# facebookresearch/omni3d

Hardware: AMD Instinct MI355X
Metric: images/sec train DLA34_FPN b=4/GPU (higher is better)
Workload: dtype f32; 1 GPU; cubercnn_DLA34_FPN train step, batch 4/GPU, synthetic Omni3D 512x512 (8 GT/img), fwd+10 losses+bwd+allreduce+divergence guard+SGD, random-init weights; global_batch=4, image=512x512, parallelism=dp1 (flat-bucket RCCL all-reduce)

## Files before the change

### include/omni3d_hip.h

```cpp
#ifndef OMNI3D_HIP_H
#define OMNI3D_HIP_H

#ifdef __cplusplus
extern "C" {
#endif


int omni_iou_box3d(const float* boxes1, int N, const float* boxes2, int M, const int* valid1, float* vol,
                   float* iou, int* overflow, void* stream);

int omni_iou_box3d_pairs(const float* boxes1, const float* boxes2, const int* idx1, const int* idx2,
                         long long npairs, const int* valid1, float* vol, float* iou, int* overflow,
                         void* stream);

int omni_iou_box3d_pairs_algo(const float* boxes1, const float* boxes2, const int* idx1, const int* idx2,
                              long long npairs, const int* valid1, float* vol, float* iou, int* overflow,
                              int lanes_per_pair, void* stream);

int omni_box3d_validity(const float* boxes, int N, float eps_coplanar, float eps_nonzero, int* valid,
                        int* counts, void* stream);

int omni_nms3d(const float* verts, const float* score, const int* cls, const int* count, int B, int S, float iou_thr,
               int class_agnostic, float eps_coplanar, float eps_nonzero, float* iou, int* keep, int* order, int* new_count,
               int* overflow, void* stream);
// ... 57 lines not shown

int omni_conv2d_fwd_multi_det(const void* const* xs, const int* cs, int nsrc, const float* w, const float* bias, float* out, int N, int H,
                              int W, int K, int ldo, int relu, int tile, int splits_req, float* stats, int stats_rows, int* nblk_out,
                              float* ws, long long ws_floats, int* ctr, int n_ctr, long long* plan, void* stream);
int omni_conv2d_dgrad_det(const float* dy, const float* w, float* dx, int N, int H, int W, int C, int K, int R, int S,
                          int stride, int pad, int lddy, int lddx, int accumulate, int tile, int splits, float* ws,
                          long long ws_floats, int* ctr, int n_ctr, long long* plan, void* stream);
int omni_conv2d_wgrad_det(const float* x, const float* dy, float* dw, int N, int H, int W, int C, int K, int R, int S,
                          int stride, int pad, int ldx, int lddy, int accumulate, int tile, float* ws, long long ws_floats,
                          int* ctr, int n_ctr, long long* plan, void* stream);

int omni_gemm_batched_split(const float* A, const float* B, float* out, int batch, int M, int N, int K, int terms, void* stream);
int omni_conv2d_s2_dgrad(const float* dy, const float* w, float* dx, int N, int H, int W, int C, int K, int lddy, int lddx,
                         int accumulate, void* stream);
int omni_conv2d_wgrad_multi_det(const void* const* xs, const int* cs, int nsrc, const float* dy, float* dw, int N, int H, int W, int K,
                                int lddy, int accumulate, int tile, float* ws, long long ws_floats, int* ctr, int n_ctr, long long* plan,
                                void* stream);


int omni_bn_fwd_algo(const float* x, const float* partial, int nblk, const float* gamma, const float* beta, const float* residual,
                     float* y, long long ldy, float* running_mean, float* running_var, float* mean_rstd, float* scale_shift,
                     double* ws, int P, int C, float eps, float momentum, int relu, int fuse_rows, void* stream);
int omni_bn_bwd_algo(const float* x, const float* dy, long long lddy, const float* y, const float* gamma, const float* mean_rstd,
                     const float* partial, int nblk, float* dx, float* dres, const float* res_carry, long long ldc, float* dgamma,
                     float* dbeta, double* ws, float* coef, int P, int C, int relu, int accumulate_param_grads, int fuse_rows,
                     void* stream);

int omni_bn_apply(const float* x, const float* scale_shift, const float* residual, float* y, int P, int C,
                  int relu, void* stream);

int omni_bn_frozen_fwd(const float* x, const float* gamma, const float* beta, const float* running_mean, const float* running_var,
                       float eps, const float* residual, float* y, int P, int C, int relu, void* stream);
int omni_bn_frozen_bwd(const float* x, const float* dy, long long lddy, const float* y, const float* gamma, const float* beta,
                       const float* running_mean, const float* running_var, float eps, float* dx, float* dres, const float* res_carry,
                       long long ldc, float* dgamma, float* dbeta, float* ws, long long ws_floats, int P, int C, int relu,
                       int accumulate_param_grads, void* stream);

int omni_maxpool2_fwd(const float* x, float* y, int N, int H, int W, int C, void* stream);
int omni_maxpool2_bwd(const float* x, const float* dy, float* dx, int N, int H, int W, int C, void* stream);

int omni_grouped_conv2d_fwd(const float* x, const float* w, float* out, int N, int H, int W, int C, int K, int R, int S, int stride,
                            int pad, int groups, void* stream);
int omni_grouped_conv2d_dgrad(const float* dy, const float* w, float* dx, int N, int H, int W, int C, int K, int R, int S, int stride,
                              int pad, int groups, void* stream);
int omni_grouped_conv2d_wgrad(const float* x, const float* dy, float* dw, int N, int H, int W, int C, int K, int R, int S, int stride,
                              int pad, int groups, void* stream);

int omni_dwconv_fwd(const float* x, const float* w, float* y, int N, int H, int W, int C, int R, int stride, int pad, void* stream);
int omni_dwconv_dgrad(const float* dy, const float* w, float* dx, int N, int H, int W, int C, int R, int stride, int pad, void* stream);
int omni_dwconv_wgrad(const float* x, const float* dy, float* dw, int N, int H, int W, int C, int R, int stride, int pad, void* stream);

int omni_avgpool2_fwd(const float* x, float* y, int N, int H, int W, int C, void* stream);
int omni_avgpool2_bwd(const float* dy, float* dx, int N, int H, int W, int C, void* stream);

int omni_subsample2_fwd(const float* x, float* y, int N, int H, int W, int C, void* stream);
int omni_subsample2_bwd(const float* dy, float* dx, int N, int H, int W, int C, void* stream);

int omni_upsample2_add(const float* lat, const float* top, float* out, int N, int H, int W, int C,
                       void* stream);
int omni_upsample2_bwd(const float* dout, float* dtop, int N, int H, int W, int C, void* stream);

int omni_wino_out_carry(const float* M, const float* carry, long long ldc, float* y, int N, int H, int W, int K, int tile, void* stream);
int omni_maxpool2_bwd_carry(const float* x, const float* dy, long long lddy, const float* carry, long long ldc, float* dx, int N, int H,
                            int W, int C, void* stream);
int omni_subsample2_bwd_carry(const float* dy, const float* carry, long long ldc, float* dx, int N, int H, int W, int C, void* stream);
int omni_upsample2_bwd_carry(const float* dout, const float* carry, long long ldc, float* dtop, int N, int H, int W, int C,
                             void* stream);

int omni_preprocess(const unsigned char* img, float* out, int N, int H, int W, int PH, int PW, float m0,
                    float m1, float m2, float s0, float s1, float s2, void* stream);
int omni_preprocess_masked(const unsigned char* img, const int* image_hw, float* out, int N, int H, int W, int PH, int PW,
                           float m0, float m1, float m2, float s0, float s1, float s2, void* stream);
int omni_preprocess_multi(const void* const* imgs, const int* image_hw, float* out, int N, int H, int W, int PH, int PW, float m0,
                          float m1, float m2, float s0, float s1, float s2, void* stream);


int omni_topk_rows(const float* keys, int rows, int n, long long pitch, int estride, int k, float* out_val,
                   int* out_idx, void* stream);
int omni_topk_segments(const float* keys, int rows, long long pitch, int estride, int nseg, const int* seg_off,
                       const int* seg_n, int k, float* out_val, int* out_idx, void* stream);

int omni_nms_sorted(const float* boxes, const int* counts, const int* valid, int Q, int nmax, float iou_thr,
                    unsigned long long* mask_ws, int* keep, void* stream);


int omni_pairwise_iou(const float* boxes1, int N, const float* boxes2, int M, int mode, float* out, void* stream);


int omni_rpn_finalize_labels(const float* anchors, int A, int B, const int* gt_off, const float* ign,
                             const int* ign_off, const signed char* match_label, const int* gt_best_idx,
                             const float* pos_val, const int* pos_idx, const float* neg_val, const int* neg_idx,
                             int kpos, int kneg, int batch_per_image, float ignore_thresh, signed char* labels,
                             int* counts, void* stream);

int omni_rpn_gather_logits(const void* const* level_ptrs, const int* level_hw, int nlev, int B, float* logits,
                           void* stream);

int omni_rpn_head16_fwd(const void* const* t, const long long* pix, int nlev, const float* w_obj, const float* b_obj,
                        const float* w_del, const float* b_del, const void* const* y, void* stream);
int omni_rpn_head16_dgrad(const void* const* dy, const void* const* t, const long long* pix, int nlev, const float* w_obj,
                          const float* w_del, int relu_mask, const void* const* dt, void* stream);
int omni_rpn_head16_wgrad(const void* const* dy, const void* const* t, const long long* pix, int nlev, float* partial,
                          int partial_rows, float* dw_obj, float* db_obj, float* dw_del, float* db_del, int accumulate, void* stream);

int omni_rpn_loss_fwd(const void* const* level_ptrs, const int* level_hw, int nlev, int B, const float* anchors,
                      const signed char* labels, const int* matched_idx, const float* gt, const int* gt_off,
                      double* sums, void* stream);
int omni_rpn_loss_bwd(const void* const* level_ptrs, const void* const* dlevel_ptrs, const int* level_hw, int nlev,
                      int B, const float* anchors, const signed char* labels, const int* matched_idx,
                      const float* gt, const int* gt_off, const float* g_cls, const float* g_loc, float inv_norm,
                      void* stream);

int omni_rpn_loss_plain_fwd(const void* const* level_ptrs, const int* level_hw, int nlev, int B, const float* anchors,
                            const signed char* labels, const int* matched_idx, const float* gt, const int* gt_off,
                            double* sums, void* stream);
int omni_rpn_loss_plain_bwd(const void* const* level_ptrs, const void* const* dlevel_ptrs, const int* level_hw, int nlev,
                            int B, const float* anchors, const signed char* labels, const int* matched_idx,
                            const float* gt, const int* gt_off, const float* g_cls, const float* g_loc, float inv_norm,
                            void* stream);

int omni_rpn_decode(const void* const* level_ptrs, const int* level_hw, int nlev, int B, int Ktot,
                    const int* slot_level, const int* idx, const float* anchors, const int* image_hw,
                    float scale_clamp, float min_size, float* boxes, int* valid, void* stream);

int omni_rpn_mask_scores(const float* scores, const int* keep, long long n, float* masked, void* stream);
int omni_rpn_collect(const float* boxes, const float* top_v, const int* top_i, int B, int N, int P, float* prop,
                     int* count, void* stream);

int omni_rpn_match_draw(const float* anchors, int A, const float* gt, const int* gt_off, int B, int G, float thr_lo,
                        float thr_hi, int l0, int l1, int l2, int allow_low_quality, const float* expo, long long* draw_state,
                        int* ticket, float eps, float* matched_val, int* matched_idx, signed char* match_label, int* gt_best_bits,
                        int* gt_best_idx, float* key_pos, float* key_neg, void* stream);
int omni_roi_sample_draw(const float* prop_boxes, const int* prop_count, int B, int pmax, const float* gt, const int* gt_cls,
                         const int* gt_off, const float* ign, const int* ign_off, const float* expo, long long* draw_state, int* ticket,
                         float iou_thr, float ignore_thresh, float eps, int num_classes, int batch_per_image, int nfg_max,
                         int append_gt, float* out_boxes, int* out_cls, int* out_gt, float* out_iou, int* out_counts, int* out_row,
                         int first, float* first_boxes, int* first_cls, int* first_row, void* stream);


int omni_roi_levels(const float* rois, int R, int min_level, int max_level, float canonical_size,
                    int canonical_level, int* levels, void* stream);

int omni_roi_align_fwd(const void* const* level_ptrs, const int* level_hw, const float* level_scale, int nlev,
                       const float* rois, const int* batch_idx, const int* levels, int R, int P, int C,
                       float* out, void* stream);
int omni_roi_align_fwd_mode(const void* const* level_ptrs, const int* level_hw, const float* level_scale, int nlev,
                            const float* rois, const int* batch_idx, const int* levels, int R, int P, int C, int aligned, float* out,
                            void* stream);
int omni_roi_align_bwd_mode(const void* const* dlevel_ptrs, const int* level_hw, const float* level_scale, int nlev,
                            const float* rois, const int* batch_idx, const int* levels, int R, int P, int C, int aligned,
                            const float* dout, void* stream);
int omni_roi_pool_fwd(const void* const* level_ptrs, const int* level_hw, const float* level_scale, int nlev, const float* rois,
                      const int* batch_idx, const int* levels, int R, int P, int C, float* out, int* argmax, void* stream);
int omni_roi_pool_bwd(const void* const* dlevel_ptrs, const int* level_hw, const float* level_scale, int nlev, const int* batch_idx,
                      const int* levels, int R, int P, int C, const float* dout, const int* argmax, void* stream);
int omni_roi_align_fwd2(const void* const* level_ptrs, const int* level_hw, const float* level_scale, int nlev,
                        const float* rois, const int* batch_idx, const int* levels, int R, int P, int C, float* out,
                        float* out2, int per_image, int first, void* stream);
int omni_roi_align_bwd(const void* const* dlevel_ptrs, const int* level_hw, const float* level_scale, int nlev,
                       const float* rois, const int* batch_idx, const int* levels, int R, int P, int C,
                       const float* dout, void* stream);
int omni_roi_align_bwd2(const void* const* dlevel_ptrs, const int* level_hw, const float* level_scale, int nlev,
                        const float* rois, const int* batch_idx, const int* levels, int R, int P, int C,
                        const float* dout, const float* dout2, int per_image, int first, void* stream);
int omni_roi_align_bwd_det(const void* const* dlevel_ptrs, const int* level_hw, const float* level_scale, int nlev, int B,
                           const float* rois, const int* batch_idx, const int* levels, int R, int P, int C, const float* dout,
// ... 185 lines not shown
```

### omni3d_amd/csrc/select_nms.hip

```cpp
#include <device_rt.h>

namespace {

constexpr int TOPK_THREADS = 1024;
constexpr int TOPK_MAXK = 8192;

__device__ __forceinline__ unsigned score_bits(float f) {
    unsigned u = __float_as_uint(f);
    if (f != f) u = 0u;
    else if (f == 0.f) u = 0x80000000u;
    else u = (u & 0x80000000u) ? ~u : (u | 0x80000000u);
    return u;
}
__device__ __forceinline__ unsigned long long key_of_bits(unsigned u, int idx) {
    return ((unsigned long long)u << 32) | (unsigned long long)(0xFFFFFFFFu - (unsigned)idx);
}
__device__ __forceinline__ unsigned long long make_key(float f, int idx) { return key_of_bits(score_bits(f), idx); }
__device__ __forceinline__ void store_key(unsigned long long* sel, int slot, unsigned u, int idx) {
    unsigned* w = reinterpret_cast<unsigned*>(sel + slot);
    w[0] = 0xFFFFFFFFu - (unsigned)idx;
    w[1] = u;
}
__device__ __forceinline__ bool key_ge(unsigned u, int idx, unsigned thi, unsigned tlo) {
    return u > thi || (u == thi && (0xFFFFFFFFu - (unsigned)idx) >= tlo);
// ... 189 lines not shown
                for (int q = 0; q < 4; ++q) {
                    const unsigned long long key = ((unsigned long long)cu[q] << 32) | cl[q];
                    if (cv[q] && key >= thr) sel[atomicAdd(&s_count, 1)] = key;
                }
            }
            for (int i = kk + t; i < kpad; i += TOPK_THREADS) sel[i] = 0ull;
            selected = true;
        }
    }

    if (!selected) {
        unsigned long long thr = 0ull;
        if (kk < n) {
            if (t == 0) { R.prefix = 0ull; R.need = kk; }
            __syncthreads();
            for (int pass = 7; pass >= 0; --pass) {
                if (t < 256) R.hist[t] = 0u;
                __syncthreads();
                const unsigned long long prefix = R.prefix;
                const int shift = pass * 8;
                if (NPT > 0 && !PREF) {
                    int tt = t, nn = n;
                    OMNI_OPAQUE_V(tt);
                    OMNI_OPAQUE_S(nn);
                    const unsigned phi = (unsigned)(prefix >> 32), plo = (unsigned)prefix;
                    const bool hi = pass >= 4;
                    const int sh = hi ? shift - 32 : shift;
#pragma unroll
                    for (int j = 0; j < NPT; ++j) {
                        if (j * TOPK_THREADS >= nn) break;
                        const int i = j * TOPK_THREADS + tt;
                        const unsigned w = hi ? ku[j] : (0xFFFFFFFFu - (unsigned)i), pw = hi ? phi : plo;
                        bool todo = i < nn && (hi || ku[j] == phi);
                        if (sh < 24) todo = todo && ((w >> (sh + 8)) == (pw >> (sh + 8)));
                        count_digit(R.hist, todo, (w >> sh) & 255u);
                    }
                } else {
                    for (int base = 0; base < n; base += TOPK_THREADS) {
                        const int i = base + t;
                        bool todo = false;
                        unsigned digit = 0u;
                        if (i < n) {
                            const unsigned long long key = make_key(row[(long)i * estride], i);
                            todo = (pass == 7) || ((key >> (shift + 8)) == (prefix >> (shift + 8)));
                            digit = (unsigned)(key >> shift) & 255u;
                        }
                        count_digit(R.hist, todo, digit);
                    }
                }
                __syncthreads();
                radix_pick_bin(R, shift);
                __syncthreads();
                if (R.done) break;
            }
            thr = R.prefix;
        }
        if (t == 0) s_count = 0;
        for (int i = t; i < kpad; i += TOPK_THREADS) sel[i] = 0ull;
        __syncthreads();
        if (NPT > 0 && !PREF) {
            int tt = t;
            OMNI_OPAQUE_V(tt);
            const unsigned thi = (unsigned)(thr >> 32), tlo = (unsigned)thr;
#pragma unroll
            for (int j = 0; j < NPT; ++j) {
                if (j * TOPK_THREADS >= n) break;
                const int i = j * TOPK_THREADS + tt;
                if (i < n && key_ge(ku[j], i, thi, tlo)) {
                    const int slot = atomicAdd(&s_count, 1);
                    if (slot < TOPK_MAXK) store_key(sel, slot, ku[j], i);
                }
            }
        } else {
            for (int i = t; i < n; i += TOPK_THREADS) {
                const unsigned long long key = make_key(row[(long)i * estride], i);
                if (key >= thr) {
                    const int slot = atomicAdd(&s_count, 1);
                    if (slot < TOPK_MAXK) sel[slot] = key;
                }
            }
        }
    }
    __syncthreads();
    for (int size = 2; size <= kpad; size <<= 1) {
        for (int stride = size >> 1; stride > 0; stride >>= 1) {
            for (int i = t; i < (kpad >> 1); i += TOPK_THREADS) {
                const int lo = 2 * i - (i & (stride - 1));
                const int hi = lo + stride;
                const bool desc = ((lo & size) == 0);
                const unsigned long long a = sel[lo], b = sel[hi];
                if ((a < b) == desc) { sel[lo] = b; sel[hi] = a; }
            }
            __syncthreads();
        }
    }
    for (int i = t; i < k; i += TOPK_THREADS) {
        const long o = (long)blockIdx.x * k + i;
        if (i < kk) { out_val[o] = key_value(sel[i]); out_idx[o] = key_index(sel[i]); }
        else { out_val[o] = -INFINITY; out_idx[o] = -1; }
    }
}

__global__ void __launch_bounds__(256) nms_mask_kernel(const float* __restrict__ boxes, const int* __restrict__ counts,
                                                       int nmax, int words, float thr,
                                                       unsigned long long* __restrict__ mask) {
    const int lane = threadIdx.x & 63, wave = threadIdx.x >> 6;
    const int q = blockIdx.z, rb = blockIdx.y * 4 + wave, cb = blockIdx.x;
    const int n = counts ? counts[q] : nmax;
    if ((int)blockIdx.y * 4 > cb || cb * 64 >= n) return;
    __shared__ float cbx[64 * 4];
    const float* B = boxes + (long)q * nmax * 4;
    if (wave == 0) {
        const int j = cb * 64 + lane;
        if (j < n) {
            cbx[lane * 4 + 0] = B[j * 4 + 0]; cbx[lane * 4 + 1] = B[j * 4 + 1];
            cbx[lane * 4 + 2] = B[j * 4 + 2]; cbx[lane * 4 + 3] = B[j * 4 + 3];
        }
    }
    __syncthreads();
    if (cb < rb || rb * 64 >= n) return;
    const int i = rb * 64 + lane;
    if (i >= n) return;
    const float x1 = B[i * 4 + 0], y1 = B[i * 4 + 1], x2 = B[i * 4 + 2], y2 = B[i * 4 + 3];
    const float ai = (x2 - x1) * (y2 - y1);
    unsigned long long bits = 0ull;
    const int jmax = (n - cb * 64) < 64 ? (n - cb * 64) : 64;
    for (int jj = (rb == cb ? lane + 1 : 0); jj < jmax; ++jj) {
        const float u1 = cbx[jj * 4 + 0], v1 = cbx[jj * 4 + 1], u2 = cbx[jj * 4 + 2], v2 = cbx[jj * 4 + 3];
        const float w = fmaxf(fminf(x2, u2) - fmaxf(x1, u1), 0.f);
        const float h = fmaxf(fminf(y2, v2) - fmaxf(y1, v1), 0.f);
        const float inter = w * h;
        const float aj = (u2 - u1) * (v2 - v1);
        const float iou = inter / (ai + aj - inter);
        if (iou > thr) bits |= (1ull << jj);
    }
    mask[((long)q * nmax + i) * words + cb] = bits;
}

constexpr int SCAN_WAVES = 16;
template <int NMS_SCAN_WAVES>
__global__ void __launch_bounds__(64 * NMS_SCAN_WAVES) nms_scan_kernel(const unsigned long long* __restrict__ mask,
                                                                       const int* __restrict__ counts, const int* __restrict__ valid,
                                                                       int nmax, int words, int* __restrict__ keep) {
    constexpr int RPW = 64 / NMS_SCAN_WAVES;
    const int q = blockIdx.x, tid = threadIdx.x, lane = tid & 63, wave = tid >> 6;
    const int n = counts ? counts[q] : nmax;
    __shared__ unsigned long long s_alive;
    __shared__ unsigned long long s_next[NMS_SCAN_WAVES];
    for (int i = n + tid; i < nmax; i += 64 * NMS_SCAN_WAVES) keep[(long)q * nmax + i] = 0;
    const int nchunks = (n + 63) / 64;
    unsigned long long rw0[RPW], rw1[RPW], diag = 0ull, acc0 = 0ull, acc1 = 0ull, removed_c = 0ull;
    int okv = 0;
    auto fetch = [&](int c) {
#pragma unroll
        for (int rr = 0; rr < RPW; ++rr) {
            const int row = c * 64 + wave * RPW + rr;
            const long rowbase = ((long)q * nmax + row) * words;
            const int w0 = lane, w1 = 64 + lane;
            rw0[rr] = (row < n && w0 > c && w0 < words && w0 * 64 < n) ? mask[rowbase + w0] : 0ull;
            rw1[rr] = (words > 64 && row < n && w1 > c && w1 < words && w1 * 64 < n) ? mask[rowbase + w1] : 0ull;
        }
        if (wave == 0) {
            const int i = c * 64 + lane;
            diag = i < n ? mask[((long)q * nmax + i) * words + c] : 0ull;
            okv = (i < n && (valid == nullptr || valid[(long)q * nmax + i] != 0)) ? 1 : 0;
        }
    };
    if (nchunks > 0) fetch(0);
    for (int c = 0; c < nchunks; ++c) {
        if (wave == 0) {
            const int i = c * 64 + lane;
            unsigned long long alive = __ballot(okv != 0) & ~removed_c;
            for (int r = 0; r < 64; ++r) {
                const unsigned long long d = __shfl(diag, r, 64);
                if ((alive >> r) & 1ull) alive &= ~d;
            }
            if (i < n) keep[(long)q * nmax + i] = (int)((alive >> lane) & 1ull);
            if (lane == 0) s_alive = alive;
        }
        __syncthreads();
        const unsigned long long alive = s_alive;
#pragma unroll
        for (int rr = 0; rr < RPW; ++rr) {
            if ((alive >> (wave * RPW + rr)) & 1ull) { acc0 |= rw0[rr]; acc1 |= rw1[rr]; }
        }
        const int nw = c + 1;
        const unsigned long long mine = __shfl(nw < 64 ? acc0 : acc1, nw & 63, 64);
        if (lane == 0) s_next[wave] = mine;
        if (c + 1 < nchunks) fetch(c + 1);
        __syncthreads();
        if (wave == 0) {
            removed_c = 0ull;
#pragma unroll
            for (int k = 0; k < NMS_SCAN_WAVES; ++k) removed_c |= s_next[k];
        }
    }
}

inline void launch_topk(int blocks, int nmax, const float* keys, const SegP& seg, long pitch, int estride, int k, float* out_val,
                        int* out_idx, hipStream_t st) {
    if (nmax <= TOPK_NPT * TOPK_THREADS && k <= TOPK_PREFILTER_K)
        hipLaunchKernelGGL(HIP_KERNEL_NAME(topk_rows_kernel<TOPK_NPT, true>), dim3(blocks), dim3(TOPK_THREADS), 0, st, keys, seg, pitch, estride,
                           k, out_val, out_idx);
    else if (nmax <= TOPK_NPT * TOPK_THREADS)
        hipLaunchKernelGGL(HIP_KERNEL_NAME(topk_rows_kernel<TOPK_NPT, false>), dim3(blocks), dim3(TOPK_THREADS), 0, st, keys, seg, pitch, estride,
                           k, out_val, out_idx);
    else
        hipLaunchKernelGGL(HIP_KERNEL_NAME(topk_rows_kernel<0, false>), dim3(blocks), dim3(TOPK_THREADS), 0, st, keys, seg, pitch, estride, k,
                           out_val, out_idx);
}

}

extern "C" {

int omni_topk_rows(const float* keys, int rows, int n, long long pitch, int estride, int k, float* out_val, int* out_idx,
                   void* stream) {
    if (rows < 0 || n < 0 || k <= 0 || k > TOPK_MAXK || estride <= 0) return OMNI_ERR_ARG;
    if (rows == 0) return OMNI_OK;
    SegP seg;
    seg.S = 1;
    for (int i = 0; i < TOPK_MAXSEG; ++i) { seg.off[i] = 0; seg.n[i] = n; }
    launch_topk(rows, n, keys, seg, (long)pitch, estride, k, out_val, out_idx, (hipStream_t)stream);
    return omni_launch_status();
}

int omni_topk_segments(const float* keys, int rows, long long pitch, int estride, int nseg, const int* seg_off,
                       const int* seg_n, int k, float* out_val, int* out_idx, void* stream) {
    if (rows < 0 || nseg <= 0 || nseg > TOPK_MAXSEG || k <= 0 || k > TOPK_MAXK || estride <= 0) return OMNI_ERR_ARG;
    if (rows == 0) return OMNI_OK;
    SegP seg;
    seg.S = nseg;
    for (int i = 0; i < TOPK_MAXSEG; ++i) {
        seg.off[i] = i < nseg ? seg_off[i] : 0;
        seg.n[i] = i < nseg ? seg_n[i] : 0;
        if (seg.off[i] < 0 || seg.n[i] < 0) return OMNI_ERR_ARG;
    }
    int nmax = 0;
    for (int i = 0; i < nseg; ++i) nmax = seg.n[i] > nmax ? seg.n[i] : nmax;
    launch_topk(rows * nseg, nmax, keys, seg, (long)pitch, estride, k, out_val, out_idx, (hipStream_t)stream);
    return omni_launch_status();
}

int omni_nms_sorted(const float* boxes, const int* counts, const int* valid, int Q, int nmax, float iou_thr,
                    unsigned long long* mask_ws, int* keep, void* stream) {
    if (Q < 0 || nmax < 0 || nmax > 8192) return OMNI_ERR_ARG;
    if (Q == 0 || nmax == 0) return OMNI_OK;
    const int words = (nmax + 63) / 64;
    hipStream_t st = (hipStream_t)stream;
    hipLaunchKernelGGL(nms_mask_kernel, dim3(words, (words + 3) / 4, Q), dim3(256), 0, st, boxes, counts, nmax, words, iou_thr,
                       mask_ws);
    hipLaunchKernelGGL(HIP_KERNEL_NAME(nms_scan_kernel<SCAN_WAVES>), dim3(Q), dim3(64 * SCAN_WAVES), 0, st, (const unsigned long long*)mask_ws,
                       counts, valid, nmax, words, keep);
    return omni_launch_status();
}

}
```

### omni3d_amd/cubercnn/modeling/proposal_generator/rpn.py

```python
import math

import torch
from torch import nn

from .... import functional as HF
from ....d2.config import configurable
from ....d2.structures import Boxes, Instances
from ....kernels import det, select
from ..anchors import build_anchor_generator
from ..layers import Conv2d
from ..registries import PROPOSAL_GENERATOR_REGISTRY, RPN_HEAD_REGISTRY

CL = torch.channels_last


@RPN_HEAD_REGISTRY.register()
class StandardRPNHead(nn.Module):

    @configurable
    def __init__(self, *, in_channels, num_anchors, box_dim=4, conv_dims=(-1,)):
        super().__init__()
        assert len(conv_dims) == 1 and num_anchors == 3 and box_dim == 4, "hot path: A=3 anchors per location"
        out_channels = in_channels if conv_dims[0] == -1 else conv_dims[0]
        self.conv = Conv2d(in_channels, out_channels, kernel_size=3, stride=1, padding=1)
# ... 53 lines not shown
            raise NotImplementedError("MI355X hot path: L1 anchor regression (BBOX_REG_LOSS_TYPE smooth_l1, SMOOTH_L1_BETA 0: Base.yaml / "
                                      "upstream defaults); the reference's IoUness losses only evaluate smooth_l1 as well (rpn.py:258-271)")
        if objectness_uncertainty.lower() not in ("iouness", "none"):
            raise NotImplementedError(f"MODEL.RPN.OBJECTNESS_UNCERTAINTY '{objectness_uncertainty}': 'IoUness' (Base.yaml:55) and 'none'")
        self.plain_objectness = objectness_uncertainty.lower() == "none"
        self.pending_logs = {}
        self.injected = None
        self.last = None

    @classmethod
    def from_config(cls, cfg, input_shape):
        in_features = cfg.MODEL.RPN.IN_FEATURES
        shapes = [input_shape[f] for f in in_features]
        return {
            "in_features": in_features, "min_box_size": cfg.MODEL.PROPOSAL_GENERATOR.MIN_SIZE,
            "nms_thresh": cfg.MODEL.RPN.NMS_THRESH, "batch_size_per_image": cfg.MODEL.RPN.BATCH_SIZE_PER_IMAGE,
            "positive_fraction": cfg.MODEL.RPN.POSITIVE_FRACTION,
            "loss_weight": {"loss_rpn_cls": cfg.MODEL.RPN.LOSS_WEIGHT,
                            "loss_rpn_loc": cfg.MODEL.RPN.BBOX_REG_LOSS_WEIGHT * cfg.MODEL.RPN.LOSS_WEIGHT},
            "box_reg_loss_type": cfg.MODEL.RPN.BBOX_REG_LOSS_TYPE, "smooth_l1_beta": cfg.MODEL.RPN.SMOOTH_L1_BETA,
            "pre_nms_topk": (cfg.MODEL.RPN.PRE_NMS_TOPK_TRAIN, cfg.MODEL.RPN.PRE_NMS_TOPK_TEST),
            "post_nms_topk": (cfg.MODEL.RPN.POST_NMS_TOPK_TRAIN, cfg.MODEL.RPN.POST_NMS_TOPK_TEST),
            "anchor_generator": build_anchor_generator(cfg, shapes),
            "anchor_thresholds": cfg.MODEL.RPN.IOU_THRESHOLDS, "anchor_labels": cfg.MODEL.RPN.IOU_LABELS,
            "head": build_rpn_head(cfg, shapes), "ignore_thresh": cfg.MODEL.RPN.IGNORE_THRESHOLD,
            "objectness_uncertainty": cfg.MODEL.RPN.OBJECTNESS_UNCERTAINTY,
        }

    @torch.no_grad()
    def label_and_sample_anchors(self, anchors, targets):
        B, A = targets.B, anchors.shape[0]
        E = self.injected["E"].to(anchors.device).float().contiguous() if (self.injected is not None and "E" in self.injected) else None
        if E is None and self.__dict__.get("_draw") is None:
            from ....kernels.glue import DrawState
            self.__dict__["_draw"] = DrawState()
        thr = self.anchor_thresholds
        m = det.rpn_match(anchors, targets.gt, targets.gt_off, E, (thr[0], thr[-1]), self.anchor_labels, True, draw=self.__dict__.get("_draw"), B=B)
        kpos = max(int(self.batch_size_per_image * self.positive_fraction), 1)
        kv, ki = select.topk_rows(m["keys"], max(kpos, self.batch_size_per_image))
        pv, pi = kv[:B, :kpos].contiguous(), ki[:B, :kpos].contiguous()
        nv, ni = kv[B:, :self.batch_size_per_image].contiguous(), ki[B:, :self.batch_size_per_image].contiguous()
        labels, counts = det.rpn_finalize_labels(anchors, targets.gt_off, targets.ign, targets.ign_off, m, pv, pi, nv, ni,
                                                 self.batch_size_per_image, self.ignore_thresh)
        return labels, m["matched_idx"]

    def losses(self, levels, anchors, labels, matched_idx, targets):
        B = targets.B
        inv_norm = 1.0 / (self.batch_size_per_image * B)
        names = ("rpn/cls", "rpn/loc")
        w = tuple(self.loss_weight.get(k, 1.0) for k in names)
        vec, sums = HF.rpn_loss(levels, anchors, labels, matched_idx, targets.gt, targets.gt_off, inv_norm, w, self.plain_objectness)
        self.pending_logs = {"rpn": (sums, B)}
        return HF.LossDict({names[0]: vec[0], names[1]: vec[1]}, vectors=[(vec, names)])

    def flush_logs(self, storage):
        if "rpn" in self.pending_logs:
            sums, B = self.pending_logs.pop("rpn")
            s = sums.tolist()
            storage.put_scalar("rpn/num_pos_anchors", s[2] / B)
            storage.put_scalar("rpn/num_neg_anchors", s[3] / B)
            if not self.plain_objectness:
                storage.put_scalar("rpn/conf_pos_anchors", s[4] / max(s[2], 1.0))
                n_other = B * self._num_anchors - s[2]
                storage.put_scalar("rpn/conf_neg_anchors", s[5] / max(n_other, 1.0))

    @torch.no_grad()
    def predict_proposals(self, levels, anchors, hw_list, image_hw):
        training = self.training
        pre, post = self.pre_nms_topk[training], self.post_nms_topk[training]
        lv = [t.detach().permute(0, 2, 3, 1) for t in levels]
        pack = det.LevelPack(lv)
        B = pack.B
        logits = det.rpn_gather_logits(pack)
        L = len(hw_list)
        kmax = min(pre, max(H * W * 3 for H, W in hw_list))
        seg_n = [H * W * 3 for H, W in hw_list]
        seg_off = [sum(seg_n[:l]) for l in range(L)]
        scores, idx = select.topk_segments(logits, seg_off, seg_n, kmax)
        scores, idx = scores.view(B, L * kmax), idx.view(B, L * kmax)
        key = (L, kmax, str(idx.device))
        if getattr(self, "_slot_key", None) != key:
            self._slot_level = torch.arange(L, dtype=torch.int32, device=idx.device).repeat_interleave(kmax).contiguous()
            self._slot_key = key
        boxes, valid = det.rpn_decode(pack, self._slot_level, idx, anchors, image_hw, self.min_box_size)
        keep = select.nms_sorted(boxes.view(B * L, kmax, 4), self.nms_thresh, None, valid.view(B * L, kmax)).view(B, L * kmax)
        masked = det.rpn_mask_scores(scores.contiguous(), keep.contiguous())
        top_v, top_i = select.topk_rows(masked, post)
        prop, count = det.rpn_collect(boxes, top_v, top_i)
        if getattr(self, "keep_candidates", False):
            self.last_candidates = {"boxes": boxes, "scores": scores, "keep": keep, "valid": valid.view(B, L * kmax), "slots_per_level": kmax}
        return prop, top_v, count

    def forward(self, images, features, gt_instances=None, targets=None):
        if targets is None and gt_instances is not None:
            from ..targets import pack_instances_cached
            targets = pack_instances_cached(gt_instances, images.image_sizes, device=images.tensor.device)
        feats = [features[f] for f in self.in_features]
        hw_list = [(f.shape[2], f.shape[3]) for f in feats]
        anchors = self.anchor_generator.grid(hw_list, feats[0].device)
        self._num_anchors = anchors.shape[0]
        levels = self.rpn_head(feats)
        if self.training:
            assert targets is not None, "RPN requires ground truth in training!"
            self.__dict__["_last_hw_list"] = hw_list
            hook = self.__dict__.get("_label_split")
            if hook is not None:
                labels, matched_idx = hook()
            else:
                labels, matched_idx = self.label_and_sample_anchors(anchors, targets)
            losses = self.losses(levels, anchors, labels, matched_idx, targets)
            self.last_labels = labels
        else:
            losses = {}
        image_hw = targets.image_hw if targets is not None else torch.tensor(
            [list(s) for s in images.image_sizes], dtype=torch.int32, device=anchors.device)
        prop, scores, count = self.predict_proposals(levels, anchors, hw_list, image_hw)
        self.last = {"boxes": prop, "scores": scores, "count": count}
        if self.injected is not None and "proposals" in self.injected:
            given = self.injected["proposals"]
            prop = torch.zeros_like(prop)
            for n, b in enumerate(given):
                prop[n, :b.shape[0]] = b.to(prop.device)
            count = torch.tensor([b.shape[0] for b in given], dtype=torch.int32, device=prop.device)
        return _PackedProposals(prop, scores, count, images.image_sizes), losses


class _PackedProposals(list):

    def __init__(self, boxes, scores, count, image_sizes):
        super().__init__()
        self.boxes, self.scores, self.count, self.image_sizes = boxes, scores, count, image_sizes
        self._done = False

    def _materialise(self):
        if not self._done:
            self._done = True
            for n, c in enumerate(self.count.tolist()):
                inst = Instances(tuple(self.image_sizes[n]))
                inst.proposal_boxes = Boxes(self.boxes[n, :c])
                inst.objectness_logits = self.scores[n, :c]
                super().append(inst)

    def __len__(self):
        return len(self.image_sizes)

    def __getitem__(self, i):
        self._materialise()
        return super().__getitem__(i)

    def __iter__(self):
        self._materialise()
        return super().__iter__()


def build_proposal_generator(cfg, input_shape):
    name = cfg.MODEL.PROPOSAL_GENERATOR.NAME
    if name == "PrecomputedProposals":
        return None
    return PROPOSAL_GENERATOR_REGISTRY.get(name)(cfg, input_shape)
```

### omni3d_amd/kernels/select.py

```python
import torch

from .. import lib as _lib


def topk_rows(keys, k, n=None, pitch=None, estride=1):
    if keys.dim() == 2 and n is None:
        rows, n = keys.shape
        pitch = keys.stride(0)
        estride = keys.stride(1) if n > 1 else 1
    else:
        rows = keys.shape[0]
    L = _lib.get()
    if not keys.is_cuda and not L.emulated:
        raise _lib.OmniHipError("omni3d_amd ops run on the GPU only")
    vals = torch.empty((rows, k), dtype=torch.float32, device=keys.device)
    idx = torch.empty((rows, k), dtype=torch.int32, device=keys.device)
    L.call("omni_topk_rows", _lib.ptr(keys), rows, n, pitch, estride, k, _lib.ptr(vals), _lib.ptr(idx),
           _lib.stream_of(keys))
    return vals, idx


def topk_segments(keys, seg_off, seg_n, k):
    import ctypes
    rows = keys.shape[0]
    L = _lib.get()
    if not keys.is_cuda and not L.emulated:
        raise _lib.OmniHipError("omni3d_amd ops run on the GPU only")
    S = len(seg_off)
    vals = torch.empty((rows, S, k), dtype=torch.float32, device=keys.device)
    idx = torch.empty((rows, S, k), dtype=torch.int32, device=keys.device)
    offs = (ctypes.c_int * S)(*[int(v) for v in seg_off])
    ns = (ctypes.c_int * S)(*[int(v) for v in seg_n])
    L.call("omni_topk_segments", _lib.ptr(keys), rows, keys.stride(0), keys.stride(1) if keys.shape[1] > 1 else 1, S,
           ctypes.cast(offs, ctypes.c_void_p), ctypes.cast(ns, ctypes.c_void_p), k, _lib.ptr(vals), _lib.ptr(idx),
           _lib.stream_of(keys))
    return vals, idx


def nms_sorted(boxes, iou_thr, counts=None, valid=None, _poison=False):
    boxes = boxes.contiguous()
    Q, nmax, _ = boxes.shape
    L = _lib.check_device(boxes, counts, valid)
    words = (nmax + 63) // 64
    ws = torch.empty(max(Q * nmax * words, 1), dtype=torch.int64, device=boxes.device)
    keep = torch.empty((Q, nmax), dtype=torch.int32, device=boxes.device)
    if _poison:
        ws.fill_(-1)
        keep.fill_(7)
    L.call("omni_nms_sorted", _lib.ptr(boxes), _lib.ptr(counts), _lib.ptr(valid), Q, nmax, float(iou_thr), _lib.ptr(ws),
           _lib.ptr(keep), _lib.stream_of(boxes))
    return keep
```

Before: 376.9 images/s.

## Fuse RPN score masking into NMS scan and speed up top-k sort and NMS kernels

The NMS scan kernel now writes score-masked outputs directly, so the separate rpn_mask_scores launch is gone, and per-level counts let it skip empty slots. The scan double-buffers mask-row fetches with buffer loads and replaces the serial 64-step diagonal loop with a ballot fixpoint iteration. The mask kernel precomputes candidate areas in LDS and avoids the division when the IoU comparison is clearly decided. The top-k bitonic sort keeps two elements in registers and does small strides with wave shuffles instead of LDS passes with barriers. These are small kernels in a large training step, and the division-free comparison and ballot fixpoint add correctness risk at edge cases.

```diff
diff --git a/include/omni3d_hip.h b/include/omni3d_hip.h
--- a/include/omni3d_hip.h
+++ b/include/omni3d_hip.h
@@ -163,6 +163,8 @@
 
 int omni_nms_sorted(const float* boxes, const int* counts, const int* valid, int Q, int nmax, float iou_thr,
                     unsigned long long* mask_ws, int* keep, void* stream);
+int omni_nms_sorted_masked(const float* boxes, const int* counts, const int* valid, int Q, int nmax, float iou_thr,
+                           unsigned long long* mask_ws, int* keep, const float* scores, float* masked, void* stream);
 
 
 int omni_pairwise_iou(const float* boxes1, int N, const float* boxes2, int M, int mode, float* out, void* stream);
diff --git a/omni3d_amd/csrc/select_nms.hip b/omni3d_amd/csrc/select_nms.hip
--- a/omni3d_amd/csrc/select_nms.hip
+++ b/omni3d_amd/csrc/select_nms.hip
@@ -295,17 +295,41 @@
         }
     }
     __syncthreads();
-    for (int size = 2; size <= kpad; size <<= 1) {
-        for (int stride = size >> 1; stride > 0; stride >>= 1) {
-            for (int i = t; i < (kpad >> 1); i += TOPK_THREADS) {
-                const int lo = 2 * i - (i & (stride - 1));
-                const int hi = lo + stride;
-                const bool desc = ((lo & size) == 0);
-                const unsigned long long a = sel[lo], b = sel[hi];
-                if ((a < b) == desc) { sel[lo] = b; sel[hi] = a; }
-            }
-            __syncthreads();
-        }
+    auto lds_pass = [&](int size, int stride) {
+        for (int i = t; i < (kpad >> 1); i += TOPK_THREADS) {
+            const int lo = 2 * i - (i & (stride - 1));
+            const int hi = lo + stride;
+            const bool desc = ((lo & size) == 0);
+            const unsigned long long a = sel[lo], b = sel[hi];
+            if ((a < b) == desc) { sel[lo] = b; sel[hi] = a; }
+        }
+        __syncthreads();
+    };
+    if (kpad <= 2 * TOPK_THREADS) {
+        const int e0 = 2 * t;
+        unsigned long long a0 = e0 < kpad ? sel[e0] : 0ull, a1 = e0 + 1 < kpad ? sel[e0 + 1] : 0ull;
+        for (int size = 2; size <= kpad; size <<= 1) {
+            const bool desc = ((e0 & size) == 0);
+            if (size >= 256) {
+                if (e0 < kpad) { sel[e0] = a0; sel[e0 + 1] = a1; }
+                __syncthreads();
+                for (int stride = size >> 1; stride >= 128; stride >>= 1) lds_pass(size, stride);
+                if (e0 < kpad) { a0 = sel[e0]; a1 = sel[e0 + 1]; }
+            }
+            for (int stride = (size >> 1) < 64 ? (size >> 1) : 64; stride >= 2; stride >>= 1) {
+                const int lm = stride >> 1;
+                const unsigned long long b0 = __shfl_xor(a0, lm, 64), b1 = __shfl_xor(a1, lm, 64);
+                const bool want_max = ((t & lm) == 0) == desc;
+                a0 = ((a0 < b0) == want_max) ? b0 : a0;
+                a1 = ((a1 < b1) == want_max) ? b1 : a1;
+            }
+            if ((a0 < a1) == desc) { const unsigned long long s = a0; a0 = a1; a1 = s; }
+        }
+        if (e0 < kpad) { sel[e0] = a0; sel[e0 + 1] = a1; }
+        __syncthreads();
+    } else {
+        for (int size = 2; size <= kpad; size <<= 1)
+            for (int stride = size >> 1; stride > 0; stride >>= 1) lds_pass(size, stride);
     }
     for (int i = t; i < k; i += TOPK_THREADS) {
         const long o = (long)blockIdx.x * k + i;
@@ -314,20 +338,25 @@
     }
 }
 
+constexpr float NMS_MARGIN = 9.5367431640625e-07f;
+constexpr unsigned NMS_T_LO = 0x0D800000u, NMS_T_HI = 0x71800000u;
 __global__ void __launch_bounds__(256) nms_mask_kernel(const float* __restrict__ boxes, const int* __restrict__ counts,
                                                        int nmax, int words, float thr,
                                                        unsigned long long* __restrict__ mask) {
+#pragma clang fp contract(off)
     const int lane = threadIdx.x & 63, wave = threadIdx.x >> 6;
     const int q = blockIdx.z, rb = blockIdx.y * 4 + wave, cb = blockIdx.x;
-    const int n = counts ? counts[q] : nmax;
+    const int n = counts ? min(max(counts[q], 0), nmax) : nmax;
     if ((int)blockIdx.y * 4 > cb || cb * 64 >= n) return;
-    __shared__ float cbx[64 * 4];
+    __shared__ float4 cbx[64];
+    __shared__ float car[64];
     const float* B = boxes + (long)q * nmax * 4;
     if (wave == 0) {
         const int j = cb * 64 + lane;
         if (j < n) {
-            cbx[lane * 4 + 0] = B[j * 4 + 0]; cbx[lane * 4 + 1] = B[j * 4 + 1];
-            cbx[lane * 4 + 2] = B[j * 4 + 2]; cbx[lane * 4 + 3] = B[j * 4 + 3];
+            const float u1 = B[j * 4 + 0], v1 = B[j * 4 + 1], u2 = B[j * 4 + 2], v2 = B[j * 4 + 3];
+            cbx[lane] = make_float4(u1, v1, u2, v2);
+            car[lane] = (u2 - u1) * (v2 - v1);
         }
     }
     __syncthreads();
@@ -336,77 +365,119 @@
     if (i >= n) return;
     const float x1 = B[i * 4 + 0], y1 = B[i * 4 + 1], x2 = B[i * 4 + 2], y2 = B[i * 4 + 3];
     const float ai = (x2 - x1) * (y2 - y1);
+    const bool shortcut = thr > 0.f;
+    const float khi = 1.f + NMS_MARGIN, klo = 1.f - NMS_MARGIN;
+    const int jmax = (n - cb * 64) < 64 ? (n - cb * 64) : 64;
     unsigned long long bits = 0ull;
-    const int jmax = (n - cb * 64) < 64 ? (n - cb * 64) : 64;
-    for (int jj = (rb == cb ? lane + 1 : 0); jj < jmax; ++jj) {
-        const float u1 = cbx[jj * 4 + 0], v1 = cbx[jj * 4 + 1], u2 = cbx[jj * 4 + 2], v2 = cbx[jj * 4 + 3];
-        const float w = fmaxf(fminf(x2, u2) - fmaxf(x1, u1), 0.f);
-        const float h = fmaxf(fminf(y2, v2) - fmaxf(y1, v1), 0.f);
+#pragma unroll 4
+    for (int jj = 0; jj < jmax; ++jj) {
+        const float4 c = cbx[jj];
+        const float aj = car[jj];
+        const float w = fmaxf(fminf(x2, c.z) - fmaxf(x1, c.x), 0.f);
+        const float h = fmaxf(fminf(y2, c.w) - fmaxf(y1, c.y), 0.f);
         const float inter = w * h;
-        const float aj = (u2 - u1) * (v2 - v1);
-        const float iou = inter / (ai + aj - inter);
-        if (iou > thr) bits |= (1ull << jj);
-    }
+        const float u = ai + aj - inter;
+        const float t = thr * u;
+        const bool ranged = shortcut & ((__float_as_uint(t) - NMS_T_LO) <= (NMS_T_HI - NMS_T_LO));
+        bool over = inter > t * khi;
+        const bool under = inter < t * klo;
+        if (!(ranged & (over | under))) over = inter / u > thr;
+        if (over) bits |= (1ull << jj);
+    }
+    if (rb == cb) bits &= ~(1ull << lane);
     mask[((long)q * nmax + i) * words + cb] = bits;
 }
 
 constexpr int SCAN_WAVES = 16;
-template <int NMS_SCAN_WAVES>
+template <int NMS_SCAN_WAVES, bool WIDE>
 __global__ void __launch_bounds__(64 * NMS_SCAN_WAVES) nms_scan_kernel(const unsigned long long* __restrict__ mask,
                                                                        const int* __restrict__ counts, const int* __restrict__ valid,
-                                                                       int nmax, int words, int* __restrict__ keep) {
+                                                                       int nmax, int words, int* __restrict__ keep,
+                                                                       const float* __restrict__ scores, float* __restrict__ masked) {
     constexpr int RPW = 64 / NMS_SCAN_WAVES;
+    constexpr int NT = 64 * NMS_SCAN_WAVES;
     const int q = blockIdx.x, tid = threadIdx.x, lane = tid & 63, wave = tid >> 6;
-    const int n = counts ? counts[q] : nmax;
+    const int n = counts ? min(max(counts[q], 0), nmax) : nmax;
     __shared__ unsigned long long s_alive;
     __shared__ unsigned long long s_next[NMS_SCAN_WAVES];
-    for (int i = n + tid; i < nmax; i += 64 * NMS_SCAN_WAVES) keep[(long)q * nmax + i] = 0;
+    __shared__ unsigned long long s_valid[128], s_keep[128];
     const int nchunks = (n + 63) / 64;
-    unsigned long long rw0[RPW], rw1[RPW], diag = 0ull, acc0 = 0ull, acc1 = 0ull, removed_c = 0ull;
-    int okv = 0;
-    auto fetch = [&](int c) {
+    const omni_rsrc_t mr = omni_make_rsrc(mask + (long)q * nmax * words, (unsigned)nmax * (unsigned)words * 8u);
+    auto load64 = [&](bool ok, int word_index) -> unsigned long long {
+        const int off = ok ? word_index * 8 : OMNI_OOB;
+        const unsigned lo = omni_bufld1(mr, off), hi = omni_bufld1(mr, ok ? off + 4 : OMNI_OOB);
+        return ((unsigned long long)hi << 32) | lo;
+    };
+    struct Rows { unsigned long long w0[RPW], w1[RPW], diag; };
+    Rows A, B;
+    auto fetch = [&](int c, Rows& R) {
+        const bool live = c < nchunks;
 #pragma unroll
         for (int rr = 0; rr < RPW; ++rr) {
             const int row = c * 64 + wave * RPW + rr;
-            const long rowbase = ((long)q * nmax + row) * words;
             const int w0 = lane, w1 = 64 + lane;
-            rw0[rr] = (row < n && w0 > c && w0 < words && w0 * 64 < n) ? mask[rowbase + w0] : 0ull;
-            rw1[rr] = (words > 64 && row < n && w1 > c && w1 < words && w1 * 64 < n) ? mask[rowbase + w1] : 0ull;
-        }
+            R.w0[rr] = load64(live && row < n && w0 > c && w0 < words && w0 * 64 < n, row * words + w0);
+            R.w1[rr] = WIDE ? load64(live && row < n && w1 > c && w1 < words && w1 * 64 < n, row * words + w1) : 0ull;
+        }
+        const int i = c * 64 + lane;
+        R.diag = load64(wave == 0 && live && i < n, i * words + c);
+    };
+    fetch(0, A);
+    fetch(1, B);
+    {
+        const omni_rsrc_t vr = omni_make_rsrc(valid ? valid + (long)q * nmax : nullptr, valid ? (unsigned)nmax * 4u : 0u);
+        unsigned flag[128 / NMS_SCAN_WAVES];
+#pragma unroll
+        for (int j = 0; j < 128 / NMS_SCAN_WAVES; ++j) {
+            const int i = (j * NMS_SCAN_WAVES + wave) * 64 + lane;
+            flag[j] = omni_bufld1(vr, i < n ? i * 4 : OMNI_OOB);
+        }
+#pragma unroll
+        for (int j = 0; j < 128 / NMS_SCAN_WAVES; ++j) {
+            const int c = j * NMS_SCAN_WAVES + wave, i = c * 64 + lane;
+            const unsigned long long ok = __ballot(i < n && (valid == nullptr || flag[j] != 0u));
+            if (lane == 0 && c < nchunks) s_valid[c] = ok;
+        }
+    }
+    __syncthreads();
+    unsigned long long acc0 = 0ull, acc1 = 0ull, removed_c = 0ull;
+    auto step = [&](int c, Rows& R) {
         if (wave == 0) {
-            const int i = c * 64 + lane;
-            diag = i < n ? mask[((long)q * nmax + i) * words + c] : 0ull;
-            okv = (i < n && (valid == nullptr || valid[(long)q * nmax + i] != 0)) ? 1 : 0;
-        }
-    };
-    if (nchunks > 0) fetch(0);
-    for (int c = 0; c < nchunks; ++c) {
-        if (wave == 0) {
-            const int i = c * 64 + lane;
-            unsigned long long alive = __ballot(okv != 0) & ~removed_c;
-            for (int r = 0; r < 64; ++r) {
-                const unsigned long long d = __shfl(diag, r, 64);
-                if ((alive >> r) & 1ull) alive &= ~d;
-            }
-            if (i < n) keep[(long)q * nmax + i] = (int)((alive >> lane) & 1ull);
-            if (lane == 0) s_alive = alive;
+            const bool ok = (((s_valid[c] & ~removed_c) >> lane) & 1ull) != 0ull;
+            const unsigned long long below = R.diag & ((1ull << lane) - 1ull);
+            unsigned long long alive = __ballot(ok), prev;
+            do {
+                prev = alive;
+                alive = __ballot(ok && (below & prev) == 0ull);
+            } while (alive != prev);
+            if (lane == 0) { s_alive = alive; s_keep[c] = alive; }
         }
         __syncthreads();
         const unsigned long long alive = s_alive;
 #pragma unroll
         for (int rr = 0; rr < RPW; ++rr) {
-            if ((alive >> (wave * RPW + rr)) & 1ull) { acc0 |= rw0[rr]; acc1 |= rw1[rr]; }
+            if ((alive >> (wave * RPW + rr)) & 1ull) { acc0 |= R.w0[rr]; acc1 |= R.w1[rr]; }
         }
         const int nw = c + 1;
         const unsigned long long mine = __shfl(nw < 64 ? acc0 : acc1, nw & 63, 64);
         if (lane == 0) s_next[wave] = mine;
-        if (c + 1 < nchunks) fetch(c + 1);
+        fetch(c + 2, R);
         __syncthreads();
         if (wave == 0) {
             removed_c = 0ull;
 #pragma unroll
             for (int k = 0; k < NMS_SCAN_WAVES; ++k) removed_c |= s_next[k];
         }
+    };
+    for (int c = 0; c + 1 < nchunks; c += 2) {
+        step(c, A);
+        step(c + 1, B);
+    }
+    if (nchunks & 1) step(nchunks - 1, A);
+    for (int i = tid; i < nmax; i += NT) {
+        const bool kept = i < n && ((s_keep[i >> 6] >> (i & 63)) & 1ull) != 0ull;
+        keep[(long)q * nmax + i] = kept ? 1 : 0;
+        if (masked != nullptr) masked[(long)q * nmax + i] = kept ? scores[(long)q * nmax + i] : -INFINITY;
     }
 }
 
@@ -455,17 +526,26 @@
     return omni_launch_status();
 }
 
-int omni_nms_sorted(const float* boxes, const int* counts, const int* valid, int Q, int nmax, float iou_thr,
-                    unsigned long long* mask_ws, int* keep, void* stream) {
-    if (Q < 0 || nmax < 0 || nmax > 8192) return OMNI_ERR_ARG;
+int omni_nms_sorted_masked(const float* boxes, const int* counts, const int* valid, int Q, int nmax, float iou_thr,
+                           unsigned long long* mask_ws, int* keep, const float* scores, float* masked, void* stream) {
+    if (Q < 0 || nmax < 0 || nmax > 8192 || (scores == nullptr) != (masked == nullptr)) return OMNI_ERR_ARG;
     if (Q == 0 || nmax == 0) return OMNI_OK;
     const int words = (nmax + 63) / 64;
     hipStream_t st = (hipStream_t)stream;
     hipLaunchKernelGGL(nms_mask_kernel, dim3(words, (words + 3) / 4, Q), dim3(256), 0, st, boxes, counts, nmax, words, iou_thr,
                        mask_ws);
-    hipLaunchKernelGGL(HIP_KERNEL_NAME(nms_scan_kernel<SCAN_WAVES>), dim3(Q), dim3(64 * SCAN_WAVES), 0, st, (const unsigned long long*)mask_ws,
-                       counts, valid, nmax, words, keep);
+    if (words > 64)
+        hipLaunchKernelGGL(HIP_KERNEL_NAME(nms_scan_kernel<SCAN_WAVES, true>), dim3(Q), dim3(64 * SCAN_WAVES), 0, st,
+                           (const unsigned long long*)mask_ws, counts, valid, nmax, words, keep, scores, masked);
+    else
+        hipLaunchKernelGGL(HIP_KERNEL_NAME(nms_scan_kernel<SCAN_WAVES, false>), dim3(Q), dim3(64 * SCAN_WAVES), 0, st,
+                           (const unsigned long long*)mask_ws, counts, valid, nmax, words, keep, scores, masked);
     return omni_launch_status();
 }
 
-}
+int omni_nms_sorted(const float* boxes, const int* counts, const int* valid, int Q, int nmax, float iou_thr,
+                    unsigned long long* mask_ws, int* keep, void* stream) {
+    return omni_nms_sorted_masked(boxes, counts, valid, Q, nmax, iou_thr, mask_ws, keep, nullptr, nullptr, stream);
+}
+
+}
diff --git a/omni3d_amd/cubercnn/modeling/proposal_generator/rpn.py b/omni3d_amd/cubercnn/modeling/proposal_generator/rpn.py
--- a/omni3d_amd/cubercnn/modeling/proposal_generator/rpn.py
+++ b/omni3d_amd/cubercnn/modeling/proposal_generator/rpn.py
@@ -159,10 +159,16 @@
         if getattr(self, "_slot_key", None) != key:
             self._slot_level = torch.arange(L, dtype=torch.int32, device=idx.device).repeat_interleave(kmax).contiguous()
             self._slot_key = key
+        ckey = (B, tuple(seg_n), kmax, str(idx.device))
+        counts = self.__dict__.setdefault("_slot_counts", {}).get(ckey)
+        if counts is None:
+            per_level = torch.cat([torch.full((1,), min(kmax, n), dtype=torch.int32, device=idx.device) for n in seg_n])
+            counts = self._slot_counts[ckey] = per_level.repeat(B).contiguous()
         boxes, valid = det.rpn_decode(pack, self._slot_level, idx, anchors, image_hw, self.min_box_size)
-        keep = select.nms_sorted(boxes.view(B * L, kmax, 4), self.nms_thresh, None, valid.view(B * L, kmax)).view(B, L * kmax)
-        masked = det.rpn_mask_scores(scores.contiguous(), keep.contiguous())
-        top_v, top_i = select.topk_rows(masked, post)
+        keep, masked = select.nms_sorted_masked(boxes.view(B * L, kmax, 4), scores.contiguous().view(B * L, kmax), self.nms_thresh,
+                                                counts, valid.view(B * L, kmax))
+        keep = keep.view(B, L * kmax)
+        top_v, top_i = select.topk_rows(masked.view(B, L * kmax), post)
         prop, count = det.rpn_collect(boxes, top_v, top_i)
         if getattr(self, "keep_candidates", False):
             self.last_candidates = {"boxes": boxes, "scores": scores, "keep": keep, "valid": valid.view(B, L * kmax), "slots_per_level": kmax}
diff --git a/omni3d_amd/kernels/select.py b/omni3d_amd/kernels/select.py
--- a/omni3d_amd/kernels/select.py
+++ b/omni3d_amd/kernels/select.py
@@ -37,16 +37,35 @@
     return vals, idx
 
 
-def nms_sorted(boxes, iou_thr, counts=None, valid=None, _poison=False):
+def _nms(boxes, iou_thr, counts, valid, scores, _poison, _ws_out=None):
     boxes = boxes.contiguous()
     Q, nmax, _ = boxes.shape
-    L = _lib.check_device(boxes, counts, valid)
+    L = _lib.check_device(boxes, counts, valid, scores)
     words = (nmax + 63) // 64
     ws = torch.empty(max(Q * nmax * words, 1), dtype=torch.int64, device=boxes.device)
     keep = torch.empty((Q, nmax), dtype=torch.int32, device=boxes.device)
+    masked = None if scores is None else torch.empty((Q, nmax), dtype=torch.float32, device=boxes.device)
     if _poison:
         ws.fill_(-1)
         keep.fill_(7)
-    L.call("omni_nms_sorted", _lib.ptr(boxes), _lib.ptr(counts), _lib.ptr(valid), Q, nmax, float(iou_thr), _lib.ptr(ws),
-           _lib.ptr(keep), _lib.stream_of(boxes))
-    return keep
+        if masked is not None:
+            masked.fill_(7.0)
+    if scores is None:
+        L.call("omni_nms_sorted", _lib.ptr(boxes), _lib.ptr(counts), _lib.ptr(valid), Q, nmax, float(iou_thr), _lib.ptr(ws),
+               _lib.ptr(keep), _lib.stream_of(boxes))
+    else:
+        L.call("omni_nms_sorted_masked", _lib.ptr(boxes), _lib.ptr(counts), _lib.ptr(valid), Q, nmax, float(iou_thr), _lib.ptr(ws),
+               _lib.ptr(keep), _lib.ptr(scores), _lib.ptr(masked), _lib.stream_of(boxes))
+    if _ws_out is not None:
+        _ws_out.append(ws)
+    return keep, masked
+
+
+def nms_sorted(boxes, iou_thr, counts=None, valid=None, _poison=False, _ws_out=None):
+    return _nms(boxes, iou_thr, counts, valid, None, _poison, _ws_out)[0]
+
+
+def nms_sorted_masked(boxes, scores, iou_thr, counts=None, valid=None, _poison=False):
+    if scores.shape != boxes.shape[:2] or scores.dtype != torch.float32:
+        raise ValueError("scores must be float32 of shape (Q, nmax)")
+    return _nms(boxes, iou_thr, counts, valid, scores, _poison)
```

After: 381.1 images/s (median of 6 runs). +1.1%, better.
